# MIMUW-RL/space-gym

Hardware: AMD Instinct MI355X
Metric: env-steps/sec at batch=65536, GoalContinuous3P-v0, 1/2/4/8 MI355X (higher is better)
Workload: dtype f32

## Files before the change

### space_gym_amd/csrc/sg_engine.hip

```cpp
#include <hip/hip_runtime.h>
#include <hip/hip_ext.h>

#include <algorithm>
#include <cmath>
#include <cstdarg>
#include <cstdio>
#include <cstdlib>
#include <cstring>
#include <limits>
#include <new>
#include <string>
#include <tuple>
#include <type_traits>
#include <utility>
#include <vector>

#include "../../include/spacegym.h"

#ifdef SG_STAMPS
constexpr int kStampSlots = 16, kStampWaves = 4096;
__device__ unsigned long long sg_dbg_stamps[kStampSlots * kStampWaves];
#ifdef SG_STAMPS_ACC_ONLY
#define SG_STAMP(slot)
#else
// ... 70 lines not shown
#define SG_PASS_DECL
#define SG_PASS(slot)
#define SG_PASS_WRITE()
#define SG_ACC_DECL
#define SG_ACC(slot)
#define SG_ACC_ADD(slot, v)
#define SG_ACC_WRITE(wave)
#define SG_REAL(slot)
#endif

#include "sg_device.hpp"
#include "sg_host_config.hpp"

using namespace sg;

struct SgBuffers {
    float4 *q0, *q1, *pl[2];
    uint2 *ctr;
    uint4 *aux;
    float4 *cshift;
    double2 *orbd;
    float4 *epq;
    uint32_t *ephi;
    unsigned long long *cnt;
};

__device__ __forceinline__ void count_hits(unsigned long long *cnt, bool hit) {
    if (!cnt) return;
    const unsigned long long m = __ballot(hit);
    if (m && (threadIdx.x & 63) == __ffsll((long long)m) - 1) atomicAdd(cnt + 2, (unsigned long long)__popcll(m));
}

struct TermList {
    uint32_t *count;
    int32_t *step_env;
    float *obs;
    uint32_t capacity;
};

constexpr int kBlock = 256;

__device__ __forceinline__ Tiling load_tiling(const SgBuffers &b, int i, uint32_t episode) {
    Tiling T;
    const uint4 a = b.aux[i];
    const float4 cs = b.cshift[i];
    T.episode = episode; T.goal_draws = a.x;
// ... 590 lines not shown
    }
    struct Next {
        Tiling T;
        ShipInit s;
        float px[N], py[N], gx, gy;
    };
    __device__ __forceinline__ static float2 kept_orbit(const SgBuffers &, int) { return make_float2(0.0f, 0.0f); }
    __device__ __forceinline__ static float2 reset_orbit(const SgDev &) { return make_float2(0.0f, 0.0f); }
    __device__ __forceinline__ static void next(const SgDev &c, int env, uint32_t episode, float2, Next &n) {
        n.T.episode = episode;
        goal_reset<N>(c, c.env_index_base + (uint32_t)env, n.T, n.s, n.px, n.py, n.gx, n.gy);
    }
    __device__ __forceinline__ void install(const SgDev &c, const SgBuffers &b, int env, uint32_t episode, const Next &n, Env &e,
                                            float (&o)[D]) const {
        e.x = n.s.x; e.y = n.s.y; e.th = n.s.th; e.vx = n.s.vx; e.vy = n.s.vy; e.om = n.s.om; e.gx = n.gx; e.gy = n.gy;
#pragma unroll
        for (int j = 0; j < N; j++) { e.px[j] = n.px[j]; e.py[j] = n.py[j]; }
        store_goal_ship<N>(b, env, e);
        store_goal_planets<N>(b, env, e);
        store_tiling(b, env, n.T);
        b.ctr[env] = make_uint2(0u, episode);
        goal_observe<N>(c, e, o);
    }
    __device__ __forceinline__ static void empty_queue(const SgBuffers &b, int env, uint32_t episode) { b.ephi[env] = episode; }
    __device__ __forceinline__ static void restart_group(const SgDev &c, const SgBuffers &b, int env, uint32_t episode, int sub,
                                                         float *obs, float2) {
        Env ne;
        goal_restart_group<N>(c, b, env, episode, sub, obs, ne);
    }
    __device__ __forceinline__ static void resample(const SgDev &c, const SgBuffers &b, int env, uint32_t episode) {
        Tiling T = load_tiling(b, env, episode);
        float gx, gy;
        goal_resample(c, c.env_index_base + (uint32_t)env, T, gx, gy);
        reinterpret_cast<float2 *>(b.q1 + env)[1] = make_float2(gx, gy);
        b.aux[env] = pack_aux(T);
    }
    __device__ __forceinline__ static void resample_wave(const SgDev &c, const SgBuffers &b, int i, bool want, uint32_t episode) {
        const unsigned long long need = __ballot(want);
        if (!need) return;
        const int lane = threadIdx.x & 63, grp = lane >> 3, sub = lane & (kGroup - 1);
        const int n_items = __popcll(need), wave_env0 = i - lane;
        for (int base = 0; base < n_items; base += 64 / kGroup) {
            const int item = base + grp;
            const int src = nth_set_lane(need, item < n_items ? item : 0);
            const uint32_t ep = __shfl(episode, src);
            if (item < n_items && sub == 0) resample(c, b, wave_env0 + src, ep);
        }
    }
};

template <int N, bool ACCEL>
__global__ __launch_bounds__(kBlock) void goal_step_kernel(const SgDev *__restrict__ cfg, SgBuffers b, int n_subtiles,
                                                          const void *__restrict__ actions, float *__restrict__ obs,
                                                          float *__restrict__ reward, uint8_t *__restrict__ done,
                                                          uint8_t *__restrict__ truncated, float *__restrict__ terminal_obs,
                                                          int stream_out) {
    step_subtiles<GoalStep<N, ACCEL>>(cfg, b, n_subtiles, actions, obs, reward, done, truncated, terminal_obs, stream_out);
}

template <int N>
struct SpareEpisode {
    static constexpr int kFields = 6 + 2 * N + 2 + 7;
    __device__ __forceinline__ static void put(float *base, int slot, int tid, const ShipInit &s, const float (&px)[N],
                                               const float (&py)[N], float gx, float gy, const Tiling &T) {
        float *p = base + (slot * kFields) * kBlock + tid;
        int f = 0;
        auto w = [&](float v) { p[(f++) * kBlock] = v; };
        w(s.x); w(s.y); w(s.th); w(s.vx); w(s.vy); w(s.om); w(gx); w(gy);
#pragma unroll
        for (int j = 0; j < N; j++) { w(px[j]); w(py[j]); }
        const uint4 a = pack_aux(T);
        w(__uint_as_float(a.y)); w(__uint_as_float(a.z)); w(__uint_as_float(a.w));
        w(T.cs0); w(T.cs1); w(T.cs2); w(T.cs3);
    }
    __device__ __forceinline__ static void put_record(float *base, int slot, int tid, const float4 (&r)[6]) {
        float *p = base + (slot * kFields) * kBlock + tid;
        int f = 0;
        auto w = [&](float v) { p[(f++) * kBlock] = v; };
        w(r[0].x); w(r[0].y); w(r[0].z); w(r[0].w); w(r[1].x); w(r[1].y); w(r[1].z); w(r[1].w);
        w(r[2].x); w(r[2].y); w(r[2].z); w(r[2].w);
        if constexpr (N > 2) { w(r[3].x); w(r[3].y); }
        if constexpr (N > 3) { w(r[3].z); w(r[3].w); }
        w(r[4].x); w(r[4].y); w(r[4].z);
        w(r[5].x); w(r[5].y); w(r[5].z); w(r[5].w);
    }
    __device__ __forceinline__ static void get(const float *base, int slot, int tid, GoalEnv<N> &e, uint4 &aux, float4 &cs) {
        const float *p = base + (slot * kFields) * kBlock + tid;
        int f = 0;
        auto r = [&]() { return p[(f++) * kBlock]; };
        e.x = r(); e.y = r(); e.th = r(); e.vx = r(); e.vy = r(); e.om = r(); e.gx = r(); e.gy = r();
#pragma unroll
        for (int j = 0; j < N; j++) { e.px[j] = r(); e.py[j] = r(); }
        aux.x = 0u;
        aux.y = __float_as_uint(r()); aux.z = __float_as_uint(r()); aux.w = __float_as_uint(r());
        cs.x = r(); cs.y = r(); cs.z = r(); cs.w = r();
    }
};

template <int N, bool ACCEL, int kSpare>
__global__ __launch_bounds__(kBlock) __attribute__((amdgpu_waves_per_eu(2))) void goal_rollout_kernel(const SgDev *__restrict__ cfg, SgBuffers b, int n_steps,
                                                             const void *__restrict__ actions, float *__restrict__ obs,
                                                             float *__restrict__ reward, uint8_t *__restrict__ done,
                                                             uint8_t *__restrict__ truncated, TermList tl) {
    __shared__ float spare[kSpare * SpareEpisode<N>::kFields * kBlock];
    const SgDev &c = *cfg;
    const bool discrete = c.discrete_actions != 0;
    constexpr int D = 7 + 2 * N + 2;
// ... 73 lines not shown
        b.ctr[i] = ct;
        b.aux[i] = aux;
        b.cshift[i] = cs;
    }
}

constexpr int kPairBlock = 2 * kBlock;
#ifndef SG_RING
#define SG_RING 5
#endif
constexpr int kRing = SG_RING;
constexpr int kHand = 9;
constexpr int kReplayCap = 128;
#ifndef SG_REPLAY_AT
#define SG_REPLAY_AT 56
#endif
#ifndef SG_PILOT_SLEEP
#define SG_PILOT_SLEEP 40
#endif
constexpr int kReplayAt = SG_REPLAY_AT;
constexpr uint32_t kSpinLimit = 1u << 21;

constexpr int kQDepth = 4;
constexpr int kQCols = 6;
template <int N>
struct EpisodeQueue {
    __device__ __forceinline__ static float4 *slot(float4 *q, int64_t B, int i, uint32_t episode) {
        return q + ((episode % (uint32_t)kQDepth) * (uint32_t)kQCols * (uint32_t)B + (uint32_t)i);
    }
    __device__ __forceinline__ static void put(float4 *q, int64_t B, int i, const ShipInit &s, const float (&px)[N],
                                               const float (&py)[N], float gx, float gy, const Tiling &T) {
        float4 *p = slot(q, B, i, T.episode);
        p[0] = make_float4(s.x, s.y, s.th, s.vx);
        p[B] = make_float4(s.vy, s.om, gx, gy);
        p[2 * B] = make_float4(px[0], py[0], px[1], py[1]);
        if constexpr (N == 3) p[3 * B] = make_float4(px[2], py[2], 0.0f, 0.0f);
        if constexpr (N == 4) p[3 * B] = make_float4(px[2], py[2], px[3], py[3]);
        const uint4 a = pack_aux(T);
        p[4 * B] = make_float4(__uint_as_float(a.y), __uint_as_float(a.z), __uint_as_float(a.w), 0.0f);
        p[5 * B] = make_float4(T.cs0, T.cs1, T.cs2, T.cs3);
    }
};

__device__ __forceinline__ uint32_t flag_load(const uint32_t *p) {
    return __hip_atomic_load(p, __ATOMIC_ACQUIRE, __HIP_MEMORY_SCOPE_WORKGROUP);
}
__device__ __forceinline__ void flag_store(uint32_t *p, uint32_t v) {
    __hip_atomic_store(p, v, __ATOMIC_RELEASE, __HIP_MEMORY_SCOPE_WORKGROUP);
}
__device__ __forceinline__ uint32_t lds_flag_load(const uint32_t *p) {
    const uint32_t v = __hip_atomic_load(p, __ATOMIC_RELAXED, __HIP_MEMORY_SCOPE_WORKGROUP);
    __builtin_amdgcn_fence(__ATOMIC_ACQUIRE, "workgroup", "local");
    return v;
}
__device__ __forceinline__ uint32_t lds_flag_peek(const uint32_t *p) {
    return __hip_atomic_load(p, __ATOMIC_RELAXED, __HIP_MEMORY_SCOPE_WORKGROUP);
}
__device__ __forceinline__ void lds_flag_store(uint32_t *p, uint32_t v) {
    __builtin_amdgcn_fence(__ATOMIC_RELEASE, "workgroup", "local");
    __hip_atomic_store(p, v, __ATOMIC_RELAXED, __HIP_MEMORY_SCOPE_WORKGROUP);
}
__device__ __forceinline__ uint32_t lds_flag_load_uniform(const uint32_t *p) {
// ... 756 lines not shown

template <int N>
struct GoalRestore {
    static constexpr int D = 7 + 2 * N + 2;
    __device__ __forceinline__ static void observe(const SgDev &c, const EnvRecord &r, float (&o)[D]) {
        GoalEnv<N> e;
        e.x = r.q0.x; e.y = r.q0.y; e.th = r.q0.z; e.vx = r.q0.w; e.vy = r.q1.x; e.om = r.q1.y; e.gx = r.q1.z; e.gy = r.q1.w;
        e.px[0] = r.pl0.x; e.py[0] = r.pl0.y; e.px[1] = r.pl0.z; e.py[1] = r.pl0.w;
        if constexpr (N > 2) { e.px[2] = r.pl1.x; e.py[2] = r.pl1.y; }
        if constexpr (N > 3) { e.px[3] = r.pl1.z; e.py[3] = r.pl1.w; }
        goal_observe<N>(c, e, o);
    }
};
struct KeplerRestore {
    static constexpr int D = 10;
    __device__ __forceinline__ static void observe(const SgDev &c, const EnvRecord &r, float (&o)[D]) {
        KeplerEnv e;
        e.x = r.q0.x; e.y = r.q0.y; e.th = r.q0.z; e.vx = r.q0.w; e.vy = r.q1.x; e.om = r.q1.y; e.phi = r.q1.z; e.ecc = r.q1.w;
        kepler_observe(c, e, o);
    }
};

template <typename F>
__device__ __forceinline__ void restore_envs(const SgDev *cfg, uint32_t *ephi, StateCols h, StateCols s, const DevSnapHeader *hdr,
                                             DevSnapHeader want, const uint8_t *mask, const int32_t *src, float *obs, uint8_t *sel,
                                             uint32_t *epoch, int *status) {
    const int i = blockIdx.x * kBlock + threadIdx.x;
    const DevSnapHeader hd = *hdr;
    if (hd.magic != want.magic || hd.family != want.family || hd.n_planets != want.n_planets ||
        hd.randomize_orbit != want.randomize_orbit || hd.num_envs != want.num_envs || hd.flags != want.flags) {
        if (i == 0) *status = kStatusSnapshot;
        if (sel && i < want.num_envs) sel[i] = 0;
        return;
    }
    if (i == 0 && epoch) *epoch += kRenderRestoreEpoch;
    const bool chosen = i < want.num_envs && (!mask || mask[i] != 0);
    int j = i;
    if (chosen && src) j = src[i];
    const bool take = chosen && (uint32_t)j < (uint32_t)want.num_envs;
    if (chosen && !take) *status = kStatusSnapshot;
    if (sel && i < want.num_envs) sel[i] = take;
    if (!__ballot(take)) return;
    if (!take) return;
    const EnvRecord r = copy_env(h, s, j, h, i);
    if (ephi) ephi[i] = r.ctr.y;
    if (obs) {
        float o[F::D];
        F::observe(*cfg, r, o);
        store_row(obs, i, o);
    }
}
template <int N>
__global__ __launch_bounds__(kBlock) void goal_restore_kernel(const SgDev *__restrict__ cfg, uint32_t *__restrict__ ephi, StateCols h,
                                                             StateCols s, const DevSnapHeader *__restrict__ hdr, DevSnapHeader want,
                                                             const uint8_t *__restrict__ mask, const int32_t *__restrict__ src,
                                                             float *__restrict__ obs, uint8_t *__restrict__ sel,
                                                             uint32_t *__restrict__ epoch, int *__restrict__ status) {
    restore_envs<GoalRestore<N>>(cfg, ephi, h, s, hdr, want, mask, src, obs, sel, epoch, status);
}
__global__ __launch_bounds__(kBlock) void kepler_restore_kernel(const SgDev *__restrict__ cfg, uint32_t *__restrict__ ephi, StateCols h,
                                                               StateCols s, const DevSnapHeader *__restrict__ hdr, DevSnapHeader want,
                                                               const uint8_t *__restrict__ mask, const int32_t *__restrict__ src,
                                                               float *__restrict__ obs, uint8_t *__restrict__ sel,
                                                               uint32_t *__restrict__ epoch, int *__restrict__ status) {
    restore_envs<KeplerRestore>(cfg, ephi, h, s, hdr, want, mask, src, obs, sel, epoch, status);
}

template <bool ACCEL>
__global__ __launch_bounds__(kBlock) void kepler_rollout_kernel(const SgDev *__restrict__ cfg, SgBuffers b, int n_steps,
                                                               const void *__restrict__ actions, float *__restrict__ obs,
                                                               float *__restrict__ reward, uint8_t *__restrict__ done,
                                                               uint8_t *__restrict__ truncated, TermList tl) {
    const SgDev &c = *cfg;
    const bool discrete = c.discrete_actions != 0;
    const int i = blockIdx.x * kBlock + threadIdx.x;
    const bool live = i < c.num_envs;
    const int ii = live ? i : 0;
    const int64_t B = c.num_envs;
    KeplerEnv e;
    load_kepler_env(b, ii, e);
    uint2 ct = b.ctr[ii];
    float2 a_next = load_action_raw(discrete, actions, ii);
    for (int t = 0; t < n_steps; t++) {
        const float2 a = decode_action(discrete, a_next);
        if (t + 1 < n_steps) a_next = load_action_raw(discrete, actions, (int64_t)(t + 1) * B + ii);
        kepler_step_body<ACCEL>(c, b, i, ii, live, e, ct, a, obs + (int64_t)t * B * 10, reward + (int64_t)t * B,
                               done + (int64_t)t * B, truncated + (int64_t)t * B, nullptr, tl.count ? &tl : nullptr, t);
    }
// ... 122 lines not shown
        px[0] = p0.x; py[0] = p0.y; px[1] = p0.z; py[1] = p0.w;
        if (c.n_planets > 2) { const float4 p1 = b.pl[1][i]; px[2] = p1.x; py[2] = p1.y; px[3] = p1.z; py[3] = p1.w; }
#define SG_VF(NP)                                                                                                              \
    {                                                                                                                         \
        float cx[NP], cy[NP];                                                                                                 \
        for (int k = 0; k < NP; k++) { cx[k] = px[k]; cy[k] = py[k]; }                                                        \
        if (acc) vector_field<NP, NP, true>(c, q0.x, q0.y, q0.z, q0.w, q1.x, q1.y, a0, a1, cx, cy, f);                        \
        else vector_field<NP, NP, false>(c, q0.x, q0.y, q0.z, q0.w, q1.x, q1.y, a0, a1, cx, cy, f);                           \
    }
        if (c.n_planets == 2) SG_VF(2) else if (c.n_planets == 3) SG_VF(3) else SG_VF(4)
#undef SG_VF
    } else {
        const float cx[1] = {0.0f}, cy[1] = {0.0f};
        if (acc) vector_field<1, 1, true>(c, q0.x, q0.y, q0.z, q0.w, q1.x, q1.y, a0, a1, cx, cy, f);
        else vector_field<1, 1, false>(c, q0.x, q0.y, q0.z, q0.w, q1.x, q1.y, a0, a1, cx, cy, f);
    }
    float *o = out + 6 * i;
#pragma unroll
    for (int k = 0; k < 6; k++) o[k] = f[k];
}

__global__ __launch_bounds__(kBlock) void queue_clear_kernel(const SgDev *__restrict__ cfg, SgBuffers b) {
    const int i = blockIdx.x * kBlock + threadIdx.x;
    if (i < cfg->num_envs) b.ephi[i] = b.ctr[i].y;
}

__global__ __launch_bounds__(kBlock) void term_compact_kernel(const SgDev *__restrict__ cfg, const uint8_t *__restrict__ done_row,
                                                             const float *__restrict__ tobs, int t, int D, TermList tl) {
    const int i = blockIdx.x * kBlock + threadIdx.x;
    const bool want = i < cfg->num_envs && done_row[i < cfg->num_envs ? i : 0] != 0;
    const unsigned long long m = __ballot(want);
    if (!m) return;
    const int lane = threadIdx.x & 63, leader = __ffsll((long long)m) - 1;
    uint32_t base = 0;
    if (lane == leader) base = atomicAdd(tl.count, (uint32_t)__popcll(m));
    base = __shfl(base, leader);
    const uint32_t idx = base + (uint32_t)__popcll(m & ((1ull << lane) - 1ull));
    if (want && idx < tl.capacity) {
        tl.step_env[2 * (int64_t)idx] = t; tl.step_env[2 * (int64_t)idx + 1] = i;
        for (int k = 0; k < D; k++) tl.obs[(int64_t)idx * D + k] = tobs[(int64_t)i * D + k];
    }
}

__global__ __launch_bounds__(kBlock) void count_flags_kernel(const uint8_t *__restrict__ done, const uint8_t *__restrict__ trunc, int64_t n,
                                                            unsigned long long *cnt) {
    if (blockIdx.x == 0 && threadIdx.x == 0) atomicAdd(cnt + 3, (unsigned long long)n);
    unsigned int nd = 0, nt = 0;
// ... 962 lines not shown
    const char *sk = getenv("SPACEGYM_STEP_KERNEL");
    e->step_kernel = sk ? (!strcmp(sk, "single") ? 1 : !strcmp(sk, "pair") ? 2 : 0) : 0;
    const char *rk = getenv("SPACEGYM_ROLLOUT_KERNEL");
    e->rollout_kernel = rk ? (!strcmp(rk, "single") ? 1 : !strcmp(rk, "pair") ? 2 : 0) : 0;
    const size_t B = (size_t)d.num_envs, D = (size_t)obs_dim(d);
    const size_t NP = d.family == SG_FAMILY_GOAL ? (size_t)d.n_planets : 0;
    hipError_t st = hipSuccess;
    auto ok = [&](hipError_t r) { if (st == hipSuccess) st = r; };
    ok(hipStreamCreateWithFlags(&e->stream, hipStreamNonBlocking));
    ok(hipEventCreateWithFlags(&e->join_event, hipEventDisableTiming));
    ok(hipHostMalloc((void **)&e->h_status, sizeof(int), hipHostMallocMapped));
    if (st == hipSuccess) { *e->h_status = 0; ok(hipHostGetDevicePointer((void **)&e->d_status, e->h_status, 0)); }
    ok(dmalloc(&e->d_cfg, 1));
    ok(dmalloc(&e->d_buf, 1));
    ok(dmalloc(&e->d_cnt, 4));
    ok(dmalloc(&e->buf.q0, B)); ok(dmalloc(&e->buf.q1, B));
    ok(dmalloc(&e->buf.ctr, B)); ok(dmalloc(&e->buf.aux, B));
    if (d.family == SG_FAMILY_GOAL) {
        ok(dmalloc(&e->buf.pl[0], B));
        if (d.n_planets > 2) ok(dmalloc(&e->buf.pl[1], B));
        ok(dmalloc(&e->buf.cshift, B));
        ok(dmalloc(&e->buf.epq, (size_t)kQDepth * kQCols * B));
        ok(dmalloc(&e->buf.ephi, B));
    } else if (d.randomize_orbit) {
        ok(dmalloc(&e->buf.orbd, B));
    }
    ok(dmalloc(&e->d_actions, 2 * B)); ok(dmalloc(&e->d_obs, D * B)); ok(dmalloc(&e->d_tobs, D * B));
    ok(dmalloc(&e->d_reward, B)); ok(dmalloc(&e->d_done, B)); ok(dmalloc(&e->d_trunc, B));
    ok(dmalloc(&e->d_ship, 6 * B)); ok(dmalloc(&e->d_goal, 2 * B)); ok(dmalloc(&e->d_elapsed, B));
    if (NP) ok(dmalloc(&e->d_planets, 2 * NP * B));
    {
        auto up = [](size_t x) { return (x + 15) & ~(size_t)15; };
        e->pack_tobs = up(sizeof(float) * D * B);
        e->pack_reward = e->pack_tobs + up(sizeof(float) * D * B);
        e->pack_done = e->pack_reward + up(sizeof(float) * B);
        e->pack_trunc = e->pack_done + up(B);
        e->pack_bytes = e->pack_base_bytes = e->pack_trunc + up(B);
        const char *ho = getenv("SPACEGYM_HOST_OUT");
        e->host_out = ho ? (!strcmp(ho, "coarse") ? 1 : !strcmp(ho, "copy") ? 0 : 2) : 2;
        e->h_pack_dev[0] = e->h_pack_dev[1] = nullptr;
        ok(hipEventCreateWithFlags(&e->step_event, hipEventDisableTiming));
    }
    if (st == hipSuccess) {
        ok(hipMemsetAsync(e->buf.q0, 0, B * sizeof(float4), e->stream));
        ok(hipMemsetAsync(e->buf.q1, 0, B * sizeof(float4), e->stream));
        ok(hipMemsetAsync(e->buf.ctr, 0, B * sizeof(uint2), e->stream));
        ok(hipMemsetAsync(e->buf.aux, 0, B * sizeof(uint4), e->stream));
        if (e->buf.ephi) ok(hipMemsetAsync(e->buf.ephi, 0, B * sizeof(uint32_t), e->stream));
        ok(hipMemsetAsync(e->d_cnt, 0, 4 * sizeof(unsigned long long), e->stream));
        ok(hipStreamSynchronize(e->stream));
        ok(hipMemcpy(e->d_cfg, &e->dev, sizeof(SgDev), hipMemcpyHostToDevice));
        ok(hipMemcpy(e->d_buf, &e->buf, sizeof(SgBuffers), hipMemcpyHostToDevice));
    }
    if (st != hipSuccess) {
        int rc = fail(nullptr, SG_ERR_HIP, "sg_create: %s", hipGetErrorString(st));
        sg_destroy(e);
        return rc;
    }
    *out = e;
    return SG_OK;
}

extern "C" int sg_create_sharded(const sg_config *cfg, int n_devices, const int *devices, sg_env **out) {
    return sg_create_sharded_ex(cfg, nullptr, n_devices, devices, out);
}
extern "C" int sg_create_sharded_ex(const sg_config *cfg, const sg_params *params, int n_devices, const int *devices, sg_env **out) {
    if (!cfg || !out || !devices || n_devices <= 0) return fail(nullptr, SG_ERR_INVALID, "sg_create_sharded: bad argument");
    for (int k = 0; k < n_devices; k++) out[k] = nullptr;
    const int64_t base = cfg->num_envs / n_devices, rem = cfg->num_envs % n_devices;
    if (base <= 0) return fail(nullptr, SG_ERR_INVALID, "sg_create_sharded: fewer envs than devices");
    int64_t lo = 0;
    for (int k = 0; k < n_devices; k++) {
        sg_config c = *cfg;
        c.num_envs = base + (k < rem ? 1 : 0);
        c.env_index_base = cfg->env_index_base + (uint32_t)lo;
        const int rc = sg_create_ex(&c, params, devices[k], &out[k]);
        if (rc) {
            for (int j = 0; j < k; j++) { sg_destroy(out[j]); out[j] = nullptr; }
            return rc;
        }
        lo += c.num_envs;
    }
    return SG_OK;
}

extern "C" int sg_destroy(sg_env *e) {
    if (!e) return SG_OK;
    (void)hipSetDevice(e->device);
    if (e->stream) { (void)join_device_work(e); (void)hipStreamSynchronize(e->stream); }
    for (auto &p : e->prof_events) { (void)hipEventDestroy(p.first); (void)hipEventDestroy(p.second); }
    void *ptrs[] = {e->buf.q0, e->buf.q1, e->buf.pl[0], e->buf.pl[1], e->buf.ctr, e->buf.aux,
                    e->buf.cshift, e->buf.orbd, e->buf.epq, e->buf.ephi, e->d_cfg, e->d_buf, e->d_actions, e->d_obs, e->d_reward, e->d_tobs,
                    e->d_ship, e->d_planets, e->d_goal, e->d_done, e->d_trunc, e->d_elapsed, e->d_pack, e->d_cnt,
                    e->d_ep_ret, e->d_ep_len, e->d_epo_ret, e->d_epo_len,
                    e->d_nstate, e->d_returns, e->d_npart, e->d_nmtab, e->d_nstab, e->d_nsel,
                    e->d_rslots, e->d_rtrace, e->d_rprims, e->d_rverts, e->d_rcounts, e->d_rids, e->d_repoch, e->d_rframes,
                    e->d_ptab, e->d_pidx};
    for (void *p : ptrs)
        if (p) (void)hipFree(p);
    for (void *p : e->norm_retired) (void)hipFree(p);
    for (uint8_t *p : e->h_pack)
        if (p) (void)hipHostFree(p);
    if (e->step_event) (void)hipEventDestroy(e->step_event);
    if (e->h_status) (void)hipHostFree(e->h_status);
    if (e->join_event) (void)hipEventDestroy(e->join_event);
    if (e->stream) (void)hipStreamDestroy(e->stream);
    delete e;
    return SG_OK;
}

extern "C" int sg_get_params(const sg_env *e, sg_params *p) {
    if (!e || !p) return SG_ERR_INVALID;
    sg_params_init(p);
    const SgDev &d = e->dev;
    p->max_engine_force = d.max_engine_force; p->ship_moi = 1.0 / (double)d.inv_moi;
// ... 1218 lines not shown
    dev_snapshot_cols(e, snap_dev, &s);
    snapshot_kernel<<<grid_for(e), kBlock, 0, (hipStream_t)hip_stream>>>(handle_cols(e), s, dev_snapshot_header(e),
                                                                        static_cast<DevSnapHeader *>(snap_dev));
    SG_HIP(e, hipGetLastError());
    note_device_work(e, (hipStream_t)hip_stream);
    return SG_OK;
}

extern "C" int sg_restore_device(sg_env *e, const void *snap_dev, size_t bytes, const uint8_t *mask_dev, const int32_t *src_dev,
                                 float *obs_dev, void *hip_stream) {
    if (!e) return SG_ERR_INVALID;
    int rc = dev_snapshot_check(e, snap_dev, bytes, "sg_restore_device");
    if (rc) return rc;
    hipStream_t s = (hipStream_t)hip_stream;
    StateCols sc;
    dev_snapshot_cols(e, const_cast<void *>(snap_dev), &sc);
    const StateCols h = handle_cols(e);
    const DevSnapHeader want = dev_snapshot_header(e);
    const DevSnapHeader *hdr = static_cast<const DevSnapHeader *>(snap_dev);
    const bool norm = obs_dev && e->d_nstate && e->norm.obs;
    uint8_t *sel = norm ? e->d_nsel : nullptr;
    uint32_t *epoch = e->d_rslots ? e->d_repoch : nullptr;
    const int grid = grid_for(e);
#define SG_RESTORE_ARGS e->d_cfg, e->buf.ephi, h, sc, hdr, want, mask_dev, src_dev, obs_dev, sel, epoch, e->d_status
    if (e->dev.family == SG_FAMILY_GOAL) {
        switch (e->dev.n_planets) {
            case 2: goal_restore_kernel<2><<<grid, kBlock, 0, s>>>(SG_RESTORE_ARGS); break;
            case 3: goal_restore_kernel<3><<<grid, kBlock, 0, s>>>(SG_RESTORE_ARGS); break;
            default: goal_restore_kernel<4><<<grid, kBlock, 0, s>>>(SG_RESTORE_ARGS); break;
        }
    } else {
        kepler_restore_kernel<<<grid, kBlock, 0, s>>>(SG_RESTORE_ARGS);
    }
#undef SG_RESTORE_ARGS
    SG_HIP(e, hipGetLastError());
    if (norm) {
        const int B = (int)e->dev.num_envs, D = obs_dim(e->dev), S = D + 1;
        norm_merge_kernel<<<D, kBlock, 0, s>>>(B, S, 1, 0, e->d_npart, e->d_nstate, e->d_nmtab, e->d_nstab, e->norm.epsilon, 1);
        const int64_t n = (int64_t)B * D;
        const int ga = (int)std::min<int64_t>((n + kBlock - 1) / kBlock, 1024);
        norm_apply_masked_kernel<<<ga, kBlock, 0, s>>>(B, D, obs_dev, sel, e->d_nmtab, e->d_nstab, e->norm.clip_obs);
        SG_HIP(e, hipGetLastError());
    }
    note_device_work(e, s);
    return SG_OK;
}

// ... 569 lines not shown
```

### space_gym_amd/csrc/sg_goal_pair_rollout.inc

```

    const SgBuffers &b = *bufs;
    using Spare = SpareEpisode<N>;
    using Queue = EpisodeQueue<N>;
    using Integ = Integrator<N, N, true, ACCEL>;
    using Replay = GoalReplay<N>;
    __shared__ float spare[kSpare * Spare::kFields * kBlock];
    __shared__ float ring[kRing * kHand * kBlock];
    __shared__ float rbuf[(kBlock / 64) * Replay::kWords * kReplayCap];
    __shared__ uint32_t spare_hi[kBlock];
    __shared__ uint32_t handed[kBlock / 64], taken[kBlock / 64];
    __shared__ uint32_t rp_tail[kBlock / 64];
    __shared__ uint32_t rp_claim[kBlock / 64], rp_done[kBlock / 64];
    constexpr int D = 7 + 2 * N + 2;
    SG_REAL(0);
    const int tid = threadIdx.x & (kBlock - 1), pair = tid >> 6, lane = tid & 63;
    const bool pilot = threadIdx.x < kBlock;
    const int i = blockIdx.x * kBlock + tid;
    const bool live = i < num_envs;
    const int ii = live ? i : 0;
    const int64_t B = num_envs;
    GoalEnv<N> e;
    load_goal_env<N>(b, ii, e);
    uint2 ct = b.ctr[ii];
    const SgDev &c = *cfg;
    {
        const uint32_t *cw = reinterpret_cast<const uint32_t *>(cfg);
        uint32_t touch = 0u;
#pragma unroll
        for (int k = 0; k < (int)(sizeof(SgDev) / 4); k += 16) touch ^= cw[k];
        touch ^= cw[sizeof(SgDev) / 4 - 1];
// ... 2 lines not shown
    const bool discrete = c.discrete_actions != 0;
    float *const rb = rbuf + pair * Replay::kWords * kReplayCap;
    if (!pilot) spare_hi[tid] = ct.y;
    if (threadIdx.x < kBlock / 64) { handed[threadIdx.x] = 0u; taken[threadIdx.x] = 0u; rp_tail[threadIdx.x] = 0u; rp_claim[threadIdx.x] = 0u; rp_done[threadIdx.x] = 0u; }
    __syncthreads();
    SG_REAL(1);

    if (pilot) {
        SG_ACC_DECL;
        __builtin_amdgcn_s_setprio(3);
        const bool hand_over = c.auto_reset && live;
        const bool auto_reset = c.auto_reset != 0;
        StepConsts kc = step_consts(c);
        asm volatile("" : "+v"(kc.max_engine_force), "+v"(kc.h), "+v"(kc.half_world), "+v"(kc.gm), "+v"(kc.omega_limit), "+v"(kc.planet_r),
                          "+v"(kc.max_thruster_force), "+v"(kc.inv_moi), "+v"(kc.planet_r_d));
        int max_steps = c.max_episode_steps;
        asm volatile("" : "+v"(max_steps));
        float2 a_next = load_action_raw(discrete, actions, ii);
        uint32_t taken_seen = 0u;
        uint32_t head = 0u, tail_seen = 0u;
        for (int t = 0; t < n_steps; t++) {
            const float2 a = decode_action(discrete, a_next);
            if (t + 1 < n_steps) a_next = load_action_raw(discrete, actions, (int64_t)(t + 1) * B + ii);
            if (t - (int)taken_seen >= kRing && !wait_flag<SG_PILOT_SLEEP>(&taken[pair], (uint32_t)(t - kRing + 1), &taken_seen)) { *status = 1; break; }
            if (head + 64u - tail_seen > (uint32_t)kReplayCap) tail_seen = lds_flag_load_uniform(&rp_tail[pair]);
            const bool defer = hand_over && head + 64u - tail_seen <= (uint32_t)kReplayCap;

            const int slot = t % kRing;
            StepResult r;
            int rk;
            {
                Integ I;
                SG_ACC(0);
                goal_env_begin<N, ACCEL>(kc, e, a.x, a.y, I);
                SG_ACC(1);
                rk = I.run(r, [&]() __attribute__((always_inline)) -> bool { return defer; });
                SG_ACC_ADD(7, __any(r.done) ? 1 : 0);
                SG_ACC_ADD(10, __any(r.path == kPathScipyErr || r.path == kPathScipyClear) ? 1 : 0);
                SG_ACC_ADD(11, __any((r.path == kPathScipyErr || r.path == kPathScipyClear) && r.n_rk > 1) ? 1 : 0);
                SG_ACC(2);
            }
            const bool replayed = rk == kRkEventDeferred;
            uint32_t rslot = 0u;
            {
                const unsigned long long dm = __ballot(replayed);
                if (dm) {
                    rslot = (head + (uint32_t)__popcll(dm & ((1ull << lane) - 1ull))) % (uint32_t)kReplayCap;
                    if (replayed) Replay::put(rb, rslot, ((uint32_t)t << 6) | (uint32_t)lane, e, a);
                    head += (uint32_t)__popcll(dm);
                }
            }
// ... 59 lines not shown
        SG_REAL(3);
        return;
    }

    SG_ACC_DECL;
    const bool auto_reset = c.auto_reset != 0;
    const int wave_env0 = i - lane;
    unsigned long long *const cnt = b.cnt;
    GoalStepConsts fc = goal_step_consts(c);
#if SG_ROLLOUT_PROFILED
    {
        const GoalRewardView v = rs.goal(c, ii);
        fc.danger_r2 = v.danger_r2; fc.survival = v.survival; fc.goal_scale = v.goal_scale; fc.safety_scale = v.safety_scale;
        fc.sparse = v.sparse;
    }
#endif
    asm volatile("" : "+v"(fc.goal_r2), "+v"(fc.danger_r2), "+v"(fc.survival), "+v"(fc.goal_scale), "+v"(fc.safety_scale),
                      "+v"(fc.sparse), "+v"(fc.planet_r), "+v"(fc.two_over_world));
    int max_steps = c.max_episode_steps;
    asm volatile("" : "+v"(max_steps));
    uint32_t hi = ct.y;
    uint4 aux = b.aux[ii];
    float4 cs = b.cshift[ii];
    if (auto_reset) {
        const uint32_t q_hi = b.ephi[ii];
        const int n_have = live ? min(max((int32_t)(q_hi - ct.y), 0), kSpare) : 0;
        float4 rec[kSpare][kQCols];
#pragma unroll
        for (int s = 0; s < kSpare; s++)
            if (s < n_have) {
                const float4 *p = Queue::slot(b.epq, B, i, ct.y + 1u + (uint32_t)s);
#pragma unroll
                for (int col = 0; col < kQCols; col++)
                    if (col != 3 || N > 2) rec[s][col] = p[(uint32_t)col * (uint32_t)B];
            }
#pragma unroll
        for (int s = 0; s < kSpare; s++)
            if (s < n_have) Spare::put_record(spare, (int)((ct.y + 1u + (uint32_t)s) % (uint32_t)kSpare), tid, rec[s]);
        hi = ct.y + (uint32_t)n_have;
        lds_flag_store(&spare_hi[tid], hi);
    }
    auto refill = [&]() {
        SG_ACC_ADD(10, 1);
        if (live && hi - ct.y < (uint32_t)kSpare) {
            Tiling T;
            T.episode = hi + 1u;
            ShipInit s;
            float px[N], py[N], gx, gy;
            goal_reset<N>(c, c.env_index_base + (uint32_t)i, T, s, px, py, gx, gy);
            Spare::put(spare, (int)(T.episode % (uint32_t)kSpare), tid, s, px, py, gx, gy, T);
            Queue::put(b.epq, B, i, s, px, py, gx, gy, T);
            hi = T.episode;
            lds_flag_store(&spare_hi[tid], hi);
        }
    };
    constexpr uint32_t kKeep = 1u;
    if (auto_reset && __any(live && hi - ct.y < kKeep)) refill();
    uint32_t tail = 0u, complete = 0u;
    bool mine = true;
    typedef __attribute__((address_space(1))) float gfloat;
    typedef __attribute__((address_space(1))) uint8_t gbyte;
    gfloat *obs_p = (gfloat *)obs + (int64_t)ii * D, *rew_p = (gfloat *)reward + ii;
    gbyte *done_p = (gbyte *)done + ii, *trunc_p = (gbyte *)truncated + ii;
    asm volatile("" : "+v"(obs_p), "+v"(rew_p), "+v"(done_p), "+v"(trunc_p));
    for (int t = 0; t < n_steps; t++) {
        SG_ACC(0);
        if (!wait_flag(&handed[pair], (uint32_t)(t + 1))) { *status = 2; break; }
        SG_ACC(1);
        double dXd, dYd;
        float th, vx, vy, om;
        int dn;
        bool replayed;
        {
            const int slot = t % kRing;
            const float *q = ring + (slot * kHand) * kBlock + tid;
            const uint64_t ux = (uint64_t)__float_as_uint(q[0 * kBlock]) | ((uint64_t)__float_as_uint(q[1 * kBlock]) << 32);
            const uint64_t uy = (uint64_t)__float_as_uint(q[2 * kBlock]) | ((uint64_t)__float_as_uint(q[3 * kBlock]) << 32);
            dXd = __longlong_as_double((long long)ux); dYd = __longlong_as_double((long long)uy);
            th = q[4 * kBlock]; vx = q[5 * kBlock]; vy = q[6 * kBlock]; om = q[7 * kBlock];
            const uint32_t w8 = __float_as_uint(q[8 * kBlock]);
            dn = (int)(w8 & 1u);
            replayed = (w8 & 2u) != 0u;
            if (replayed) Replay::put_goal(rb, w8 >> 8, e.gx, e.gy);
            complete += (uint32_t)__popcll(__ballot(replayed));
        }
        lds_flag_store(&taken[pair], (uint32_t)(t + 1));
        SG_ACC(3);
        float o[D], r;
        int hit;
        r = goal_reward<N>(fc, e.x, e.y, dXd, dYd, e.px, e.py, e.gx, e.gy, hit);
        count_hits(cnt, live && hit && !replayed);
        e.x = (float)((double)e.x + dXd); e.y = (float)((double)e.y + dYd); e.vx = vx; e.vy = vy; e.om = om; e.th = th;
        const uint32_t el = ct.x + 1u;
        const int trunc = !dn && (int)el >= max_steps;
        const int fin = dn | trunc;
        const bool restart = live && fin && auto_reset;
        if (live) ct.x = el;
        SG_ACC(4);
        if constexpr (TOBS) {
            if (__any(restart && !replayed)) {
                goal_observe<N>(fc, e, o);
                term_append<D>(tl, restart && !replayed, t, i, o);
            }
        }
        const uint32_t keep = t + 1 < n_steps ? kKeep : 0u;
        if (auto_reset && __any(live && hi - ct.y < (restart ? keep + 1u : keep))) refill();
        SG_ACC(6);
        if (restart) {
            ct = make_uint2(0u, ct.y + 1u);
            Spare::get(spare, (int)(ct.y % (uint32_t)kSpare), tid, e, aux, cs);
        }
        SG_ACC(12);
        goal_observe<N>(fc, e, o);
        SG_ACC(13);
        if (live) {
#pragma unroll
            for (int k = 0; k < D; k++) obs_p[k] = o[k];
            if (!replayed) *rew_p = r;
            *done_p = (uint8_t)fin;
            *trunc_p = (uint8_t)trunc;
        }
        obs_p += B * D; rew_p += B; done_p += B; trunc_p += B;
        asm volatile("" : "+v"(obs_p), "+v"(rew_p), "+v"(done_p), "+v"(trunc_p));
        SG_ACC(5);
        SG_ACC(7);
        SG_ACC_ADD(11, __any(live && hit && !restart) ? 1 : 0);
        if (live && hit && !restart) {
            Tiling T;
            T.episode = ct.y; T.goal_draws = aux.x;
            T.ship_tile = aux.y & 0xffu; T.goal_tile = (aux.y >> 8) & 0xffu; T.case_b = (aux.y >> 16) & 1u; T.flip = (aux.y >> 17) & 1u;
            T.free_counts = (uint64_t)aux.z | ((uint64_t)aux.w << 32);
            T.cs0 = cs.x; T.cs1 = cs.y; T.cs2 = cs.z; T.cs3 = cs.w;
            goal_resample(c, c.env_index_base + (uint32_t)i, T, e.gx, e.gy);
            aux = pack_aux(T);
        }
        SG_ACC(2);
        if (complete - tail >= (uint32_t)kReplayAt && mine) {
            const uint32_t n = min(complete - tail, 64u);
            uint32_t got = 0u;
            if (lane == 0) got = atomicCAS(&rp_claim[pair], tail, tail + n);
            mine = (uint32_t)__builtin_amdgcn_readfirstlane((int)got) == tail;
            if (mine) {
                __builtin_amdgcn_fence(__ATOMIC_ACQ_REL, "workgroup", "local");
                goal_replay_pass<N, ACCEL, TOBS>(c, rb, tail, n, lane, wave_env0, B, reward, tl, &rp_tail[pair], cnt SG_ROLLOUT_RS);
                tail += n;
            }
        }
        SG_ACC(9);
    }
    SG_ACC_WRITE(blockIdx.x * 8 + 4 + pair);
    SG_REAL(2);
    if (live) {
        reinterpret_cast<float2 *>(b.q1 + i)[1] = make_float2(e.gx, e.gy);
        b.aux[i] = aux;
        b.cshift[i] = cs;
        if (auto_reset) b.ephi[i] = hi;
    }
    if (tail != complete) {
        if (!wait_flag(&rp_done[pair], 1u)) *status = 3;
#pragma unroll 1
        while (tail != complete) {
            const uint32_t n = min(complete - tail, 64u);
            goal_replay_reward<N, TOBS>(c, rb, tail, n, lane, wave_env0, B, reward, tl, cnt SG_ROLLOUT_RS);
            tail += n;
        }
    }
    SG_REAL(3);
```

Before: 29.35 billion.

## Precompute first goal resample at episode generation to skip on-hit resampling

When a spare episode is generated, the first goal resample is drawn ahead of time and its tile bits and coordinates are stored in the spare LDS slot, the episode queue (an extra column) and a new per-env epg buffer. On the first goal hit of an episode the rollout takes the precomputed goal instead of running goal_resample inline, which takes that divergent work off the per-step critical path. For N=4 the LDS ring depth is capped at 4 to offset the larger spare footprint. The cost is more LDS, more queue traffic and extra bookkeeping to clear epg on restore and queue clear.

Result: no change. 29.26 billion (-0.3%).

```diff
diff --git a/space_gym_amd/csrc/sg_engine.hip b/space_gym_amd/csrc/sg_engine.hip
--- a/space_gym_amd/csrc/sg_engine.hip
+++ b/space_gym_amd/csrc/sg_engine.hip
@@ -116,6 +116,7 @@
     double2 *orbd;
     float4 *epq;
     uint32_t *ephi;
+    uint4 *epg;
     unsigned long long *cnt;
 };
 
@@ -752,7 +753,10 @@
         b.ctr[env] = make_uint2(0u, episode);
         goal_observe<N>(c, e, o);
     }
-    __device__ __forceinline__ static void empty_queue(const SgBuffers &b, int env, uint32_t episode) { b.ephi[env] = episode; }
+    __device__ __forceinline__ static void empty_queue(const SgBuffers &b, int env, uint32_t episode) {
+        b.ephi[env] = episode;
+        b.epg[env] = make_uint4(0u, 0u, 0u, 0u);
+    }
     __device__ __forceinline__ static void restart_group(const SgDev &c, const SgBuffers &b, int env, uint32_t episode, int sub,
                                                          float *obs, float2) {
         Env ne;
@@ -788,11 +792,29 @@
     step_subtiles<GoalStep<N, ACCEL>>(cfg, b, n_subtiles, actions, obs, reward, done, truncated, terminal_obs, stream_out);
 }
 
-template <int N>
+constexpr uint32_t kAuxTilesMask = 0x3ffffu;
+constexpr int kGoal1Shift = 18;
+constexpr uint32_t kGoal1Removed = 0x100u, kGoal1Present = 0x200u, kGoal1Bits = 0x3ffu;
+__device__ __forceinline__ uint32_t goal1_draw(const SgDev &c, uint32_t env_global, const Tiling &T, float &gx1, float &gy1) {
+    Tiling T1 = T;
+    goal_resample(c, env_global, T1, gx1, gy1);
+    const bool removed = T1.free_counts != free_add(T.free_counts, T.ship_tile);
+    return (T1.goal_tile & 0xffu) | (removed ? kGoal1Removed : 0u) | kGoal1Present;
+}
+__device__ __forceinline__ uint4 goal1_take(const uint4 &aux) {
+    const uint32_t ship = aux.y & 0xffu, goal = (aux.y >> 8) & 0xffu, g1 = aux.y >> kGoal1Shift, tile1 = g1 & 0xffu;
+    uint64_t f = free_add((uint64_t)aux.z | ((uint64_t)aux.w << 32), ship);
+    if (g1 & kGoal1Removed) f = free_remove(f, tile1);
+    return make_uint4(1u, goal | (tile1 << 8) | (aux.y & 0x30000u), (uint32_t)f, (uint32_t)(f >> 32));
+}
+
+template <int N, bool G1 = false>
 struct SpareEpisode {
-    static constexpr int kFields = 6 + 2 * N + 2 + 7;
+    static constexpr int kFields = 6 + 2 * N + 2 + 7 + (G1 ? 2 : 0);
+    static constexpr int kG1Col = N == 4 ? 6 : 3;
     __device__ __forceinline__ static void put(float *base, int slot, int tid, const ShipInit &s, const float (&px)[N],
-                                               const float (&py)[N], float gx, float gy, const Tiling &T) {
+                                               const float (&py)[N], float gx, float gy, const Tiling &T, uint32_t g1 = 0u,
+                                               float gx1 = 0.0f, float gy1 = 0.0f) {
         float *p = base + (slot * kFields) * kBlock + tid;
         int f = 0;
         auto w = [&](float v) { p[(f++) * kBlock] = v; };
@@ -800,10 +822,12 @@
 #pragma unroll
         for (int j = 0; j < N; j++) { w(px[j]); w(py[j]); }
         const uint4 a = pack_aux(T);
-        w(__uint_as_float(a.y)); w(__uint_as_float(a.z)); w(__uint_as_float(a.w));
+        w(__uint_as_float(a.y | (g1 << kGoal1Shift))); w(__uint_as_float(a.z)); w(__uint_as_float(a.w));
         w(T.cs0); w(T.cs1); w(T.cs2); w(T.cs3);
-    }
-    __device__ __forceinline__ static void put_record(float *base, int slot, int tid, const float4 (&r)[6]) {
+        if constexpr (G1) { w(gx1); w(gy1); }
+    }
+    template <int C>
+    __device__ __forceinline__ static void put_record(float *base, int slot, int tid, const float4 (&r)[C]) {
         float *p = base + (slot * kFields) * kBlock + tid;
         int f = 0;
         auto w = [&](float v) { p[(f++) * kBlock] = v; };
@@ -813,6 +837,14 @@
         if constexpr (N > 3) { w(r[3].z); w(r[3].w); }
         w(r[4].x); w(r[4].y); w(r[4].z);
         w(r[5].x); w(r[5].y); w(r[5].z); w(r[5].w);
+        if constexpr (G1 && N == 4) { w(r[kG1Col].x); w(r[kG1Col].y); }
+        if constexpr (G1 && N != 4) { w(r[kG1Col].z); w(r[kG1Col].w); }
+    }
+    __device__ __forceinline__ static void get(const float *base, int slot, int tid, GoalEnv<N> &e, uint4 &aux, float4 &cs, float &gx1,
+                                               float &gy1) {
+        get(base, slot, tid, e, aux, cs);
+        const float *p = base + (slot * kFields + kFields - 2) * kBlock + tid;
+        gx1 = p[0]; gy1 = p[kBlock];
     }
     __device__ __forceinline__ static void get(const float *base, int slot, int tid, GoalEnv<N> &e, uint4 &aux, float4 &cs) {
         const float *p = base + (slot * kFields) * kBlock + tid;
@@ -932,22 +964,24 @@
 constexpr uint32_t kSpinLimit = 1u << 21;
 
 constexpr int kQDepth = 4;
-constexpr int kQCols = 6;
+constexpr int kQCols = 7;
 template <int N>
 struct EpisodeQueue {
     __device__ __forceinline__ static float4 *slot(float4 *q, int64_t B, int i, uint32_t episode) {
         return q + ((episode % (uint32_t)kQDepth) * (uint32_t)kQCols * (uint32_t)B + (uint32_t)i);
     }
     __device__ __forceinline__ static void put(float4 *q, int64_t B, int i, const ShipInit &s, const float (&px)[N],
-                                               const float (&py)[N], float gx, float gy, const Tiling &T) {
+                                               const float (&py)[N], float gx, float gy, const Tiling &T, uint32_t g1, float gx1,
+                                               float gy1) {
         float4 *p = slot(q, B, i, T.episode);
         p[0] = make_float4(s.x, s.y, s.th, s.vx);
         p[B] = make_float4(s.vy, s.om, gx, gy);
         p[2 * B] = make_float4(px[0], py[0], px[1], py[1]);
-        if constexpr (N == 3) p[3 * B] = make_float4(px[2], py[2], 0.0f, 0.0f);
-        if constexpr (N == 4) p[3 * B] = make_float4(px[2], py[2], px[3], py[3]);
+        if constexpr (N == 2) p[3 * B] = make_float4(0.0f, 0.0f, gx1, gy1);
+        if constexpr (N == 3) p[3 * B] = make_float4(px[2], py[2], gx1, gy1);
+        if constexpr (N == 4) { p[3 * B] = make_float4(px[2], py[2], px[3], py[3]); p[6 * B] = make_float4(gx1, gy1, 0.0f, 0.0f); }
         const uint4 a = pack_aux(T);
-        p[4 * B] = make_float4(__uint_as_float(a.y), __uint_as_float(a.z), __uint_as_float(a.w), 0.0f);
+        p[4 * B] = make_float4(__uint_as_float(a.y | (g1 << kGoal1Shift)), __uint_as_float(a.z), __uint_as_float(a.w), 0.0f);
         p[5 * B] = make_float4(T.cs0, T.cs1, T.cs2, T.cs3);
     }
 };
@@ -1750,7 +1784,7 @@
 };
 
 template <typename F>
-__device__ __forceinline__ void restore_envs(const SgDev *cfg, uint32_t *ephi, StateCols h, StateCols s, const DevSnapHeader *hdr,
+__device__ __forceinline__ void restore_envs(const SgDev *cfg, uint32_t *ephi, uint4 *epg, StateCols h, StateCols s, const DevSnapHeader *hdr,
                                              DevSnapHeader want, const uint8_t *mask, const int32_t *src, float *obs, uint8_t *sel,
                                              uint32_t *epoch, int *status) {
     const int i = blockIdx.x * kBlock + threadIdx.x;
@@ -1771,7 +1805,7 @@
     if (!__ballot(take)) return;
     if (!take) return;
     const EnvRecord r = copy_env(h, s, j, h, i);
-    if (ephi) ephi[i] = r.ctr.y;
+    if (ephi) { ephi[i] = r.ctr.y; epg[i] = make_uint4(0u, 0u, 0u, 0u); }
     if (obs) {
         float o[F::D];
         F::observe(*cfg, r, o);
@@ -1779,19 +1813,19 @@
     }
 }
 template <int N>
-__global__ __launch_bounds__(kBlock) void goal_restore_kernel(const SgDev *__restrict__ cfg, uint32_t *__restrict__ ephi, StateCols h,
+__global__ __launch_bounds__(kBlock) void goal_restore_kernel(const SgDev *__restrict__ cfg, uint32_t *__restrict__ ephi, uint4 *__restrict__ epg, StateCols h,
                                                              StateCols s, const DevSnapHeader *__restrict__ hdr, DevSnapHeader want,
                                                              const uint8_t *__restrict__ mask, const int32_t *__restrict__ src,
                                                              float *__restrict__ obs, uint8_t *__restrict__ sel,
                                                              uint32_t *__restrict__ epoch, int *__restrict__ status) {
-    restore_envs<GoalRestore<N>>(cfg, ephi, h, s, hdr, want, mask, src, obs, sel, epoch, status);
-}
-__global__ __launch_bounds__(kBlock) void kepler_restore_kernel(const SgDev *__restrict__ cfg, uint32_t *__restrict__ ephi, StateCols h,
+    restore_envs<GoalRestore<N>>(cfg, ephi, epg, h, s, hdr, want, mask, src, obs, sel, epoch, status);
+}
+__global__ __launch_bounds__(kBlock) void kepler_restore_kernel(const SgDev *__restrict__ cfg, uint32_t *__restrict__ ephi, uint4 *__restrict__ epg, StateCols h,
                                                                StateCols s, const DevSnapHeader *__restrict__ hdr, DevSnapHeader want,
                                                                const uint8_t *__restrict__ mask, const int32_t *__restrict__ src,
                                                                float *__restrict__ obs, uint8_t *__restrict__ sel,
                                                                uint32_t *__restrict__ epoch, int *__restrict__ status) {
-    restore_envs<KeplerRestore>(cfg, ephi, h, s, hdr, want, mask, src, obs, sel, epoch, status);
+    restore_envs<KeplerRestore>(cfg, ephi, epg, h, s, hdr, want, mask, src, obs, sel, epoch, status);
 }
 
 template <bool ACCEL>
@@ -1960,7 +1994,7 @@
 
 __global__ __launch_bounds__(kBlock) void queue_clear_kernel(const SgDev *__restrict__ cfg, SgBuffers b) {
     const int i = blockIdx.x * kBlock + threadIdx.x;
-    if (i < cfg->num_envs) b.ephi[i] = b.ctr[i].y;
+    if (i < cfg->num_envs) { b.ephi[i] = b.ctr[i].y; b.epg[i] = make_uint4(0u, 0u, 0u, 0u); }
 }
 
 __global__ __launch_bounds__(kBlock) void term_compact_kernel(const SgDev *__restrict__ cfg, const uint8_t *__restrict__ done_row,
@@ -2969,6 +3003,7 @@
         ok(dmalloc(&e->buf.cshift, B));
         ok(dmalloc(&e->buf.epq, (size_t)kQDepth * kQCols * B));
         ok(dmalloc(&e->buf.ephi, B));
+        ok(dmalloc(&e->buf.epg, B));
     } else if (d.randomize_orbit) {
         ok(dmalloc(&e->buf.orbd, B));
     }
@@ -2994,6 +3029,7 @@
         ok(hipMemsetAsync(e->buf.ctr, 0, B * sizeof(uint2), e->stream));
         ok(hipMemsetAsync(e->buf.aux, 0, B * sizeof(uint4), e->stream));
         if (e->buf.ephi) ok(hipMemsetAsync(e->buf.ephi, 0, B * sizeof(uint32_t), e->stream));
+        if (e->buf.epg) ok(hipMemsetAsync(e->buf.epg, 0, B * sizeof(uint4), e->stream));
         ok(hipMemsetAsync(e->d_cnt, 0, 4 * sizeof(unsigned long long), e->stream));
         ok(hipStreamSynchronize(e->stream));
         ok(hipMemcpy(e->d_cfg, &e->dev, sizeof(SgDev), hipMemcpyHostToDevice));
@@ -3037,7 +3073,7 @@
     if (e->stream) { (void)join_device_work(e); (void)hipStreamSynchronize(e->stream); }
     for (auto &p : e->prof_events) { (void)hipEventDestroy(p.first); (void)hipEventDestroy(p.second); }
     void *ptrs[] = {e->buf.q0, e->buf.q1, e->buf.pl[0], e->buf.pl[1], e->buf.ctr, e->buf.aux,
-                    e->buf.cshift, e->buf.orbd, e->buf.epq, e->buf.ephi, e->d_cfg, e->d_buf, e->d_actions, e->d_obs, e->d_reward, e->d_tobs,
+                    e->buf.cshift, e->buf.orbd, e->buf.epq, e->buf.ephi, e->buf.epg, e->d_cfg, e->d_buf, e->d_actions, e->d_obs, e->d_reward, e->d_tobs,
                     e->d_ship, e->d_planets, e->d_goal, e->d_done, e->d_trunc, e->d_elapsed, e->d_pack, e->d_cnt,
                     e->d_ep_ret, e->d_ep_len, e->d_epo_ret, e->d_epo_len,
                     e->d_nstate, e->d_returns, e->d_npart, e->d_nmtab, e->d_nstab, e->d_nsel,
@@ -4302,7 +4338,7 @@
     uint8_t *sel = norm ? e->d_nsel : nullptr;
     uint32_t *epoch = e->d_rslots ? e->d_repoch : nullptr;
     const int grid = grid_for(e);
-#define SG_RESTORE_ARGS e->d_cfg, e->buf.ephi, h, sc, hdr, want, mask_dev, src_dev, obs_dev, sel, epoch, e->d_status
+#define SG_RESTORE_ARGS e->d_cfg, e->buf.ephi, e->buf.epg, h, sc, hdr, want, mask_dev, src_dev, obs_dev, sel, epoch, e->d_status
     if (e->dev.family == SG_FAMILY_GOAL) {
         switch (e->dev.n_planets) {
             case 2: goal_restore_kernel<2><<<grid, kBlock, 0, s>>>(SG_RESTORE_ARGS); break;
diff --git a/space_gym_amd/csrc/sg_goal_pair_rollout.inc b/space_gym_amd/csrc/sg_goal_pair_rollout.inc
--- a/space_gym_amd/csrc/sg_goal_pair_rollout.inc
+++ b/space_gym_amd/csrc/sg_goal_pair_rollout.inc
@@ -1,11 +1,12 @@
 
     const SgBuffers &b = *bufs;
-    using Spare = SpareEpisode<N>;
+    using Spare = SpareEpisode<N, true>;
     using Queue = EpisodeQueue<N>;
     using Integ = Integrator<N, N, true, ACCEL>;
     using Replay = GoalReplay<N>;
     __shared__ float spare[kSpare * Spare::kFields * kBlock];
-    __shared__ float ring[kRing * kHand * kBlock];
+    constexpr int kRingN = N == 4 ? (kRing < 4 ? kRing : 4) : kRing;
+    __shared__ float ring[kRingN * kHand * kBlock];
     __shared__ float rbuf[(kBlock / 64) * Replay::kWords * kReplayCap];
     __shared__ uint32_t spare_hi[kBlock];
     __shared__ uint32_t handed[kBlock / 64], taken[kBlock / 64];
@@ -54,11 +55,11 @@
         for (int t = 0; t < n_steps; t++) {
             const float2 a = decode_action(discrete, a_next);
             if (t + 1 < n_steps) a_next = load_action_raw(discrete, actions, (int64_t)(t + 1) * B + ii);
-            if (t - (int)taken_seen >= kRing && !wait_flag<SG_PILOT_SLEEP>(&taken[pair], (uint32_t)(t - kRing + 1), &taken_seen)) { *status = 1; break; }
+            if (t - (int)taken_seen >= kRingN && !wait_flag<SG_PILOT_SLEEP>(&taken[pair], (uint32_t)(t - kRingN + 1), &taken_seen)) { *status = 1; break; }
             if (head + 64u - tail_seen > (uint32_t)kReplayCap) tail_seen = lds_flag_load_uniform(&rp_tail[pair]);
             const bool defer = hand_over && head + 64u - tail_seen <= (uint32_t)kReplayCap;
 
-            const int slot = t % kRing;
+            const int slot = t % kRingN;
             StepResult r;
             int rk;
             {
@@ -164,6 +165,12 @@
     uint32_t hi = ct.y;
     uint4 aux = b.aux[ii];
     float4 cs = b.cshift[ii];
+    float g1x, g1y;
+    {
+        const uint4 g = b.epg[ii];
+        g1x = __uint_as_float(g.z); g1y = __uint_as_float(g.w);
+        if (g.x == ct.y && aux.x == 0u) aux.y |= (g.y & kGoal1Bits) << kGoal1Shift;
+    }
     if (auto_reset) {
         const uint32_t q_hi = b.ephi[ii];
         const int n_have = live ? min(max((int32_t)(q_hi - ct.y), 0), kSpare) : 0;
@@ -174,7 +181,7 @@
                 const float4 *p = Queue::slot(b.epq, B, i, ct.y + 1u + (uint32_t)s);
 #pragma unroll
                 for (int col = 0; col < kQCols; col++)
-                    if (col != 3 || N > 2) rec[s][col] = p[(uint32_t)col * (uint32_t)B];
+                    if (col < 6 || N == 4) rec[s][col] = p[(uint32_t)col * (uint32_t)B];
             }
 #pragma unroll
         for (int s = 0; s < kSpare; s++)
@@ -190,8 +197,10 @@
             ShipInit s;
             float px[N], py[N], gx, gy;
             goal_reset<N>(c, c.env_index_base + (uint32_t)i, T, s, px, py, gx, gy);
-            Spare::put(spare, (int)(T.episode % (uint32_t)kSpare), tid, s, px, py, gx, gy, T);
-            Queue::put(b.epq, B, i, s, px, py, gx, gy, T);
+            float gx1, gy1;
+            const uint32_t g1 = goal1_draw(c, c.env_index_base + (uint32_t)i, T, gx1, gy1);
+            Spare::put(spare, (int)(T.episode % (uint32_t)kSpare), tid, s, px, py, gx, gy, T, g1, gx1, gy1);
+            Queue::put(b.epq, B, i, s, px, py, gx, gy, T, g1, gx1, gy1);
             hi = T.episode;
             lds_flag_store(&spare_hi[tid], hi);
         }
@@ -214,7 +223,7 @@
         int dn;
         bool replayed;
         {
-            const int slot = t % kRing;
+            const int slot = t % kRingN;
             const float *q = ring + (slot * kHand) * kBlock + tid;
             const uint64_t ux = (uint64_t)__float_as_uint(q[0 * kBlock]) | ((uint64_t)__float_as_uint(q[1 * kBlock]) << 32);
             const uint64_t uy = (uint64_t)__float_as_uint(q[2 * kBlock]) | ((uint64_t)__float_as_uint(q[3 * kBlock]) << 32);
@@ -250,7 +259,7 @@
         SG_ACC(6);
         if (restart) {
             ct = make_uint2(0u, ct.y + 1u);
-            Spare::get(spare, (int)(ct.y % (uint32_t)kSpare), tid, e, aux, cs);
+            Spare::get(spare, (int)(ct.y % (uint32_t)kSpare), tid, e, aux, cs, g1x, g1y);
         }
         SG_ACC(12);
         goal_observe<N>(fc, e, o);
@@ -266,8 +275,12 @@
         asm volatile("" : "+v"(obs_p), "+v"(rew_p), "+v"(done_p), "+v"(trunc_p));
         SG_ACC(5);
         SG_ACC(7);
-        SG_ACC_ADD(11, __any(live && hit && !restart) ? 1 : 0);
-        if (live && hit && !restart) {
+        const bool have1 = aux.x == 0u && ((aux.y >> kGoal1Shift) & kGoal1Present) != 0u;
+        SG_ACC_ADD(11, __any(live && hit && !restart && !have1) ? 1 : 0);
+        if (live && hit && !restart && have1) {
+            aux = goal1_take(aux);
+            e.gx = g1x; e.gy = g1y;
+        } else if (live && hit && !restart) {
             Tiling T;
             T.episode = ct.y; T.goal_draws = aux.x;
             T.ship_tile = aux.y & 0xffu; T.goal_tile = (aux.y >> 8) & 0xffu; T.case_b = (aux.y >> 16) & 1u; T.flip = (aux.y >> 17) & 1u;
@@ -294,8 +307,9 @@
     SG_REAL(2);
     if (live) {
         reinterpret_cast<float2 *>(b.q1 + i)[1] = make_float2(e.gx, e.gy);
-        b.aux[i] = aux;
+        b.aux[i] = make_uint4(aux.x, aux.y & kAuxTilesMask, aux.z, aux.w);
         b.cshift[i] = cs;
+        b.epg[i] = make_uint4(ct.y, aux.x == 0u ? aux.y >> kGoal1Shift : 0u, __float_as_uint(g1x), __float_as_uint(g1y));
         if (auto_reset) b.ephi[i] = hi;
     }
     if (tail != complete) {
```
